# ria8651/octree-tracer

Hardware: AMD Instinct MI355X
Metric: Mrays/sec at 1920x1080, depth-16 SVO; achieved HBM GB/s vs peak (higher is better)
Workload: dtype f32+u32

## Files before the change

include/svo_hip.h:

```cpp
#ifndef SVO_HIP_H
#define SVO_HIP_H

#include <stddef.h>
#include <stdint.h>

#ifdef __cplusplus
extern "C" {
#endif

#define SVO_VOXEL_OFFSET 134217728u

typedef enum svo_status {
    SVO_OK = 0,
    SVO_ERR_ARG = -1,
    SVO_ERR_HIP = -2,
    SVO_ERR_STATE = -3,
    SVO_ERR_NO_DEVICE = -4,
    SVO_ERR_COMM = -5,
    SVO_ERR_CAP = -6
} svo_status;

#define SVO_F_PAUSE_ADAPTIVE 1u
#define SVO_F_SHOW_STEPS 2u
#define SVO_F_SHOW_HITS 4u
// ... 19 lines not shown
typedef struct svo_ctx svo_ctx;

#define SVO_VARIANT_RESTART 0
#define SVO_VARIANT_STACK 1

typedef enum svo_option {
    SVO_OPT_VARIANT = 0,
    SVO_OPT_TIMING = 1,
    SVO_OPT_GRID_BLOCKS = 2,
    SVO_OPT_REFILL_MIN = 3,
    SVO_OPT_STRIP_ITEMS = 4,
    SVO_OPT_DYNAMIC_STRIPS = 5,
    SVO_OPT_SCHEDULE = 8,
    SVO_OPT_TREE_DEPTH = 9,
    SVO_OPT_BLOCK_SHAPE = 10,
    SVO_OPT_DEBUG_BUFFER = 7,
    SVO_OPT_SCAN_CLEARS_COUNTERS = 11,
    SVO_OPT_FUSED_SHADOWS = 12,
    SVO_OPT_PAIR_TABLE = 13,
    SVO_OPT_CULL = 14,
    SVO_OPT_CAMERA_SHORTCUT = 15,
    SVO_OPT_SCHEDULE_MOTION = 16,
    SVO_OPT_STATIC_DEAL = 17,
    SVO_OPT_PRIO_STEPS = 6
} svo_option;

int svo_device_count(void);
int svo_ctx_create(int hip_device, svo_ctx **out);
int svo_ctx_destroy(svo_ctx *ctx);
int svo_ctx_set_stream(svo_ctx *ctx, void *hip_stream, int use_own);
int svo_set_option(svo_ctx *ctx, int option, int64_t value);
const char *svo_last_error(const svo_ctx *ctx);
int svo_sync(svo_ctx *ctx);

int svo_nodes_alloc(svo_ctx *ctx, size_t capacity_words);
int svo_nodes_bind_device(svo_ctx *ctx, uint32_t *device_words, size_t capacity_words);
int svo_nodes_share(svo_ctx *ctx, svo_ctx *owner);
int svo_nodes_invalidate(svo_ctx *ctx);
int svo_nodes_write(svo_ctx *ctx, size_t word_offset, const uint32_t *host_words, size_t n);
int svo_nodes_scatter(svo_ctx *ctx, const uint32_t *indices, const uint32_t *host_words, size_t n);
int svo_nodes_read(svo_ctx *ctx, size_t word_offset, uint32_t *host_words, size_t n);
int svo_nodes_device_ptr(svo_ctx *ctx, uint32_t **out, size_t *capacity_words);

int svo_buffer_alloc(svo_ctx *ctx, size_t bytes, void **device_out);
int svo_buffer_free(svo_ctx *ctx, void *device_ptr);
int svo_buffer_read(svo_ctx *ctx, const void *device_ptr, void *host_out, size_t bytes);
// ... 23 lines not shown
int svo_comm_unique_id(uint8_t id_out[SVO_COMM_ID_BYTES]);
int svo_comm_init_rank(svo_ctx *ctx, const uint8_t id[SVO_COMM_ID_BYTES], int world, int rank);
int svo_comm_init_all(int n, svo_ctx *const *ctxs);
int svo_comm_destroy(svo_ctx *ctx);
int svo_gather_frame(svo_ctx *ctx, const void *send, size_t bytes, void *recv_on_root, int root);
int svo_gather_wait(svo_ctx *ctx);
int svo_gather_frame_all(int n, svo_ctx *const *ctxs, const void *const *send, size_t bytes, void *recv_on_root, int root);

int svo_assemble_tiles_rgba(svo_ctx *ctx, const uint32_t *gathered_rgba, uint32_t world, uint32_t n_pad, uint32_t width,
                            uint32_t height, uint32_t tile_w, uint32_t tile_h, uint32_t *rgba_frame_out);

int svo_trace_rays(svo_ctx *ctx, const float *rays, size_t n_rays, svo_hit *hits_out);

int svo_last_render_ms(svo_ctx *ctx, float *ms);
int svo_timing_collect(svo_ctx *ctx, float *ms_out, size_t cap, size_t *n_out);

int svo_diag_gather(svo_ctx *ctx, uint32_t stride_bytes, uint32_t n_loads);

int svo_diag_strip_classes(svo_ctx *ctx, uint8_t *host_out, size_t n_strips);

int svo_diag_deal(svo_ctx *ctx, uint32_t status_out[16], uint32_t *table_out, size_t table_words, uint32_t *stamps_out,
                  size_t stamps_words);

int svo_scan_dispatch(svo_ctx *ctx, uint32_t node_length);
int svo_scan_read(svo_ctx *ctx, uint32_t *sub, uint32_t *n_sub, uint32_t *unsub, uint32_t *n_unsub,
                  size_t capacity);

struct svo_cpu_octree;
struct svo_world;
typedef struct svo_proc_params {
    float pos[3];
    uint32_t base_depth;
    uint32_t chunk_depth;
    uint64_t max_nodes;
} svo_proc_params;
int svo_proc_generate_chunk(svo_ctx *ctx, const svo_proc_params *params, struct svo_cpu_octree **out);
int svo_world_generate(svo_ctx *ctx, struct svo_world *w, uint32_t world_depth, uint32_t chunk_depth);
int svo_proc_sdf(svo_ctx *ctx, const float *xyz, size_t n, float *out);
int svo_proc_classify(svo_ctx *ctx, const svo_proc_params *params, uint8_t *cells_out);
#define SVO_PROC_TIMES 10
int svo_proc_timing(svo_ctx *ctx, float ms_out[SVO_PROC_TIMES]);

typedef struct svo_build_params {
    uint32_t depth;
    uint32_t default_colour;
    uint64_t max_words;
// ... 111 lines not shown
```

octree-tracer_amd/_lib.py:

```python
import ctypes as C
import os

import torch

_HERE = os.path.dirname(os.path.abspath(__file__))
LIB_PATH = os.environ.get("SVO_HIP_LIB") or os.path.join(_HERE, "libsvo_hip.so")


class Uniforms(C.Structure):
    _fields_ = [
        ("camera", C.c_float * 16),
        ("camera_inverse", C.c_float * 16),
        ("dimensions", C.c_float * 4),
        ("sun_dir", C.c_float * 4),
        ("flags", C.c_uint32),
        ("misc_value", C.c_float),
    ]


class TerrainParams(C.Structure):
    _fields_ = [
        ("seed", C.c_uint32),
        ("max_depth", C.c_uint32),
        ("cam", C.c_float * 3),
# ... 110 lines not shown
    "svo_comm_unique_id": (C.c_int, (vp,)),
    "svo_comm_init_rank": (C.c_int, (vp, vp, C.c_int, C.c_int)),
    "svo_comm_init_all": (C.c_int, (C.c_int, C.POINTER(vp))),
    "svo_comm_destroy": (C.c_int, (vp,)),
    "svo_gather_frame": (C.c_int, (vp, vp, sz, vp, C.c_int)),
    "svo_gather_wait": (C.c_int, (vp,)),
    "svo_gather_frame_all": (C.c_int, (C.c_int, C.POINTER(vp), C.POINTER(vp), sz, vp, C.c_int)),
    "svo_set_uniforms": (C.c_int, (vp, C.POINTER(Uniforms))),
    "svo_render": (C.c_int, (vp, u32, u32, u32, u32, u32, u32, vp, vp)),
    "svo_render_host": (C.c_int, (vp, u32, u32, u32, u32, u32, u32, vp, vp)),
    "svo_render_tiles": (C.c_int, (vp, u32, u32, u32, u32, u32, u32, vp, vp)),
    "svo_render_secondary": (C.c_int, (vp, u32, u32, u32, u32, u32, u32, u32, vp, vp)),
    "svo_render_tiles_secondary": (C.c_int, (vp, u32, u32, u32, u32, u32, u32, u32, vp, vp)),
    "svo_assemble_tiles": (C.c_int, (vp, vp, u32, u32, u32, u32, u32, u32, vp)),
    "svo_assemble_tiles_packed": (C.c_int, (vp, vp, u32, u32, u32, u32, u32, u32, vp)),
    "svo_assemble_tiles_rgba": (C.c_int, (vp, vp, u32, u32, u32, u32, u32, u32, vp)),
    "svo_pack_records": (C.c_int, (vp, vp, sz, vp)),
    "svo_trace_rays": (C.c_int, (vp, vp, sz, vp)),
    "svo_last_render_ms": (C.c_int, (vp, fp)),
    "svo_timing_collect": (C.c_int, (vp, fp, sz, C.POINTER(sz))),
    "svo_diag_gather": (C.c_int, (vp, u32, u32)),
    "svo_diag_strip_classes": (C.c_int, (vp, vp, sz)),
    "svo_diag_deal": (C.c_int, (vp, vp, vp, sz, vp, sz)),
    "svo_scan_dispatch": (C.c_int, (vp, u32)),
    "svo_scan_read": (C.c_int, (vp, vp, C.POINTER(u32), vp, C.POINTER(u32), sz)),
    "svo_proc_generate_chunk": (C.c_int, (vp, C.POINTER(ProcParams), C.POINTER(vp))),
    "svo_world_generate": (C.c_int, (vp, vp, u32, u32)),
    "svo_proc_sdf": (C.c_int, (vp, vp, sz, vp)),
    "svo_proc_classify": (C.c_int, (vp, C.POINTER(ProcParams), vp)),
    "svo_proc_timing": (C.c_int, (vp, fp)),
    "svo_nodes_build": (C.c_int, (vp, vp, vp, sz, C.POINTER(BuildParams), C.POINTER(u64))),
    "svo_nodes_build_dense": (C.c_int, (vp, vp, C.POINTER(BuildParams), C.POINTER(u64))),
    "svo_buffer_write": (C.c_int, (vp, vp, vp, sz)),
    "svo_build_timing": (C.c_int, (vp, fp)),
    "svo_cpu_octree_build": (C.c_int, (vp, vp, vp, sz, C.POINTER(ChunkBuildParams), C.POINTER(vp))),
    "svo_world_build": (C.c_int, (vp, vp, vp, vp, sz, C.POINTER(ChunkBuildParams))),
    "svo_world_build_timing": (C.c_int, (vp, fp)),
    "svo_nodes_edit": (C.c_int, (vp, vp, vp, sz, C.POINTER(EditParams), C.POINTER(u64))),
    "svo_edit_timing": (C.c_int, (vp, fp)),
    "svo_nodes_compact": (C.c_int, (vp, C.POINTER(CompactParams), vp, C.POINTER(u64))),
    "svo_compact_timing": (C.c_int, (vp, fp)),
    "svo_nodes_list_voxels": (C.c_int, (vp, C.POINTER(ListParams), vp, vp, vp, C.POINTER(u64))),
    "svo_list_timing": (C.c_int, (vp, fp)),
    "svo_nodes_sample": (C.c_int, (vp, C.POINTER(SampleParams), vp, sz, vp, vp, vp)),
    "svo_nodes_sample_dense": (C.c_int, (vp, C.POINTER(SampleParams), C.POINTER(u32), C.POINTER(u32), vp)),
    "svo_sample_timing": (C.c_int, (vp, fp)),
# ... 96 lines not shown
```

octree-tracer_amd/csrc/svo_abi.cpp:

```cpp
#include <hip/hip_runtime.h>

#include <array>
#include <cmath>
#include <cstdio>
#include <cstdlib>
#include <cstring>
#include <new>
#include <string>
#include <vector>

#include "svo_ctx.h"

int svo_fail(svo_ctx *ctx, int code, const char *what) {
    if (ctx) ctx->err = what;
    return code;
}

int svo_fail_hip(svo_ctx *ctx, hipError_t e, const char *what) {
    if (ctx) ctx->err = std::string(what) + ": " + hipGetErrorString(e);
    return SVO_ERR_HIP;
}

namespace {

// ... 135 lines not shown
        }();
        HIP_TRY(ctx, hipMemcpyAsync(sc.balance, equal_shares.data(), sizeof(equal_shares), hipMemcpyHostToDevice, ctx->stream));
    }
    a.balance = plan.feed_balance ? sc.balance : nullptr;
    a.order_cap = svo::order_list_cap(n_strips);
    if (f.filtered) {
        const uint8_t *prev = plan.prior_costs ? sc.cost : nullptr;
        if (a.skip)
            HIP_TRY(ctx, svo::launch_schedule_skipping(a, prev, sc.cls_now, sc.order, n_strips, a.order_cap, ctx->stream));
        else
            HIP_TRY(ctx, svo::launch_schedule_culling(a, prev, sc.cls_now, sc.order, n_strips, a.order_cap, ctx->stream));
        a.order = sc.order;
    } else if (plan.stored_lists) {
        a.order = sc.order;
    }
    return SVO_OK;
}

int deal_before(svo_ctx *ctx, svo_ctx::Sched &sc, const svo::FrameFacts &ff, svo::TraceArgs &a, const svo::LaunchInfo &li, int sched_slot,
                svo::DealPlan &plan) {
    svo_ctx::Sched::DealBuffers &db = sc.deal;
    svo::DealFacts f;
    f.enabled = ctx->static_deal;
    f.plain_static = sched_slot == 0 && a.work.mode != 2 && a.hits && !a.skip && !a.count_nodes && !a.shadow_hits && !a.debug && !li.deep_stack;
    f.stored_lists = ff.schedule && !ff.filtered && a.order != nullptr && a.balance != nullptr;
    f.at_rest = sc.built_nodes_version == ctx->store->version && memcmp(&sc.built_uniforms, &ctx->uniforms, sizeof(svo_uniforms)) == 0;
    f.balance_frames = sc.state.balance_frames;
    if (f.enabled && f.plain_static && f.stored_lists && f.at_rest) {
        svo::LaunchInfo ask = li;
        ask.blocks_out = &f.grid_blocks;
        HIP_TRY(ctx, svo::launch_trace(a, ask, ctx->stream));
        f.row_cap = svo::deal_row_cap(a.order_cap, f.grid_blocks);
    }
    if (db.seen_pending && hipEventQuery(db.seen_ev[0]) == hipSuccess) {
        db.seen_pending = false;
        f.seen_fresh = true;
        f.seen_step = db.seen[svo::kDealStep];
        f.seen_verdict = db.seen[svo::kDealVerdict];
    }
    (void)hipGetLastError();
    const bool claimed_before = !db.last_replayed;
    plan = svo::deal_before_trace(db.state, f);
    db.last_replayed = plan.replay;
    if (plan.seed) {
        const size_t rows = (size_t)f.grid_blocks * 4;
        if (int rc = svo_grow(ctx, rows * f.row_cap, &db.table)) return rc;
        if (int rc = svo_grow(ctx, rows, &db.len)) return rc;
        if (int rc = svo_grow(ctx, svo::deal_log_words(f.grid_blocks), &db.log)) return rc;
        if (int rc = svo_grow(ctx, sc.order.size(), &db.lists)) return rc;
        if (db.stamps.size() < 2 * rows) {
            if (int rc = svo_grow(ctx, 2 * rows, &db.stamps)) return rc;
            HIP_TRY(ctx, hipMemsetAsync(db.stamps, 0, db.stamps.size() * sizeof(uint32_t), ctx->stream));
        }
        if (!db.words) {
            HIP_TRY(ctx, db.words.alloc(svo::kDealStateWords));
            HIP_TRY(ctx, db.seen.alloc(svo::kDealStateWords));
            HIP_TRY(ctx, db.seen_ev.create(hipEventDisableTiming));
            HIP_TRY(ctx, hipMemsetAsync(db.words, 0, svo::kDealStateWords * sizeof(uint32_t), ctx->stream));
            memset(db.seen, 0, svo::kDealStateWords * sizeof(uint32_t));
        }
        HIP_TRY(ctx, svo::launch_deal_seed(db.view(a.order_cap, ctx->deal_pairs_div), sc.order, claimed_before ? sc.balance.get() : nullptr, ctx->stream));
    }
    if (plan.replay) {
        a.deal_table = db.table;
        a.deal_row_cap = db.state.row_cap;
        a.deal_stamps = db.stamps;
    }
    return SVO_OK;
}

int schedule_after(svo_ctx *ctx, svo_ctx::Sched &sc, svo::FrameFacts &f, const svo::TraceArgs &a, const svo::LaunchInfo &li,
                   int sched_slot, const svo::DealPlan &deal) {
    f.same_input = (a.work.mode != 2 || sched_slot == 1) && sc.built_nodes_version == ctx->store->version &&
                   memcmp(&sc.built_uniforms, &ctx->uniforms, sizeof(svo_uniforms)) == 0;
    f.moving = sc.have_prev && memcmp(&sc.prev_uniforms, &ctx->uniforms, sizeof(svo_uniforms)) != 0;
    svo::PostPlan plan = svo::plan_after_trace(sc.state, f);
    if (deal.replay) plan.balance_update = 0u;
    HIP_TRY(ctx, svo::launch_post(a, li, plan, sc.buf(), ctx->stream));
    if (sched_slot == 0) {
        svo_ctx::Sched::DealBuffers &db = sc.deal;
        const svo::Deal view = db.view(a.order_cap, ctx->deal_pairs_div);
        if (deal.step) HIP_TRY(ctx, svo::launch_deal_step(view, sc.balance, ctx->stream));
        bool mirror = false;
        if (svo::deal_after_post(db.state, deal, plan.build_lists, mirror)) HIP_TRY(ctx, svo::launch_deal_compare(view, sc.order, ctx->stream));
        if (mirror) {
            HIP_TRY(ctx, hipMemcpyAsync(db.seen, db.words, svo::kDealStateWords * sizeof(uint32_t), hipMemcpyDeviceToHost, ctx->stream));
            HIP_TRY(ctx, hipEventRecord(db.seen_ev[0], ctx->stream));
            db.seen_pending = true;
        }
    }
    sc.prev_uniforms = ctx->uniforms;
    sc.have_prev = true;
    if (plan.rebuild) {
        sc.key = a.work;
        sc.built_uniforms = ctx->uniforms;
        sc.built_nodes_version = ctx->store->version;
    }
    return SVO_OK;
}

int trace_launch(svo_ctx *ctx, const svo::WorkDesc &work, const float *rays, svo_hit *hits, const TraceOpts &opt) {
    int rc = bind(ctx);
    if (rc) return rc;
    const bool want_stack = ctx->variant != SVO_VARIANT_RESTART && ctx->tree_depth <= (uint32_t)svo::stack_max_depth(true);
    if (want_stack) {
// ... 56 lines not shown
        ctx->defer_items = want;
    }
    li.counters = ctx->defer_buf;
    if (ctx->defer_buf) {
        uint32_t *lists = ctx->defer_buf + svo::kCounterWords;
        const size_t stride = ctx->defer_items + 1;
        li.defer = lists + (ctx->frame_parity ? stride : 0);
        li.next_defer_count = lists + (ctx->frame_parity ? 0 : stride);
    }
    svo::DealPlan deal;
    if (stack) {
        rc = deal_before(ctx, sc, f, a, li, opt.sched_slot, deal);
        if (rc) return rc;
    }
    const size_t slot = ctx->ev_slots ? (ctx->ev_count % ctx->ev_slots) : 0;
    const bool timed = ctx->ev_slots && opt.sched_slot == 0;
    if (timed) HIP_TRY(ctx, hipEventRecord(ctx->ev[slot][0], ctx->stream));
    HIP_TRY(ctx, svo::launch_trace(a, li, ctx->stream));
    if (timed) {
        HIP_TRY(ctx, hipEventRecord(ctx->ev[slot][1], ctx->stream));
        ctx->ev_count++;
    }
    if (!stack) return SVO_OK;
    rc = schedule_after(ctx, sc, f, a, li, opt.sched_slot, deal);
    if (rc) return rc;
    ctx->frame_parity ^= 1;
    return SVO_OK;
}

bool fuse_shadow_rays(const svo_ctx *ctx) {
    const bool want = ctx->fused_shadows != 0;
    if (!want || ctx->variant == SVO_VARIANT_RESTART || ctx->tree_depth > (uint32_t)svo::stack_max_depth(true)) return false;
    const float *sd = ctx->uniforms.sun_dir;
    const float sl = sqrtf((sd[0] * sd[0] + sd[1] * sd[1]) + sd[2] * sd[2]);
    for (int k = 0; k < 3; k++) {
        float d = -(sd[k] / sl);
        if (d == 0.0f) d = 0.000001f;
        if (!(fabsf(d) >= 1.0e-11f && fabsf(d) <= 2.0f)) return false;
    }
    return true;
}

int trace_common(svo_ctx *ctx, const svo::WorkDesc &work, const float *rays, svo_hit *hits, uint32_t *rgba) {
    if (!ctx->nodes) return svo_fail(ctx, SVO_ERR_STATE, "svo_nodes_alloc / svo_nodes_bind_device not called");
    if (work.mode != 2 && !ctx->have_uniforms) return svo_fail(ctx, SVO_ERR_STATE, "svo_set_uniforms not called");
    if (!hits && !rgba) return svo_fail(ctx, SVO_ERR_ARG, "both hits_out and rgba_out are NULL");
    if (!rgba) return trace_launch(ctx, work, rays, hits, TraceOpts{});
    if (work.mode == 2) return svo_fail(ctx, SVO_ERR_ARG, "explicit rays have no pixels to shade");
    int rc = bind(ctx);
// ... 310 lines not shown
                return svo_fail(ctx, SVO_ERR_ARG, "schedule motion: class floor (0..12, 0 = off) | radius (0..4) << 8 | min_count (0..80) << 12");
            ctx->motion_floor = (uint32_t)value;
            return SVO_OK;
        case SVO_OPT_CAMERA_SHORTCUT:
            ctx->cam_shortcut = value != 0;
            return SVO_OK;
        case SVO_OPT_CULL:
            if (value < 0 || value > 2) return svo_fail(ctx, SVO_ERR_ARG, "cull: 0 (off), 1 (whenever the camera is outside the cube) or 2 (automatic)");
            ctx->cull_mode = (int)value;
            return SVO_OK;
        case SVO_OPT_PAIR_TABLE:
            return SVO_OK;
        case SVO_OPT_DEBUG_BUFFER:
            ctx->debug_buf = (uint32_t *)(uintptr_t)value;
            return SVO_OK;
        case SVO_OPT_BLOCK_SHAPE:
            if (value < 0 || value > 6) return svo_fail(ctx, SVO_ERR_ARG, "block width log2 must be 0..6");
            ctx->block_w_log2 = (uint32_t)value;
            return SVO_OK;
        case SVO_OPT_PRIO_STEPS:
            if (value < 0 || value > 255) return svo_fail(ctx, SVO_ERR_ARG, "prio_steps must be 0..255");
            return SVO_OK;
        case SVO_OPT_STATIC_DEAL:
            if (value < 0 || value > 1) return svo_fail(ctx, SVO_ERR_ARG, "static deal: 0 (off) or 1 (on)");
            ctx->static_deal = value != 0;
            return SVO_OK;
        default:
            return svo_fail(ctx, SVO_ERR_ARG, "unknown option");
    }
}

const char *svo_last_error(const svo_ctx *ctx) { return ctx ? ctx->err.c_str() : "null ctx"; }

int svo_sync(svo_ctx *ctx) {
    if (!ctx) return SVO_ERR_ARG;
    int rc = bind(ctx);
    if (rc) return rc;
    HIP_TRY(ctx, hipStreamSynchronize(ctx->stream));
    if (ctx->comm_stream) HIP_TRY(ctx, hipStreamSynchronize(ctx->comm_stream));
    uint32_t st = 0;
    HIP_TRY(ctx, hipMemcpy(&st, ctx->status, sizeof(st), hipMemcpyDeviceToHost));
    if (st & 2u) {
        HIP_TRY(ctx, hipMemset(ctx->status, 0, sizeof(uint32_t)));
        return svo_fail(ctx, SVO_ERR_STATE, "fused shadow ray outside the range of the fast arithmetic (set SVO_OPT_FUSED_SHADOWS to 0)");
    }
    if (st & 1u) {
        HIP_TRY(ctx, hipMemset(ctx->status, 0, sizeof(uint32_t)));
        return svo_fail(ctx, SVO_ERR_STATE,
// ... 245 lines not shown
    if ((uint64_t)n_loads * (stride_bytes / 4) > ctx->capacity) return svo_fail(ctx, SVO_ERR_ARG, "pattern exceeds the node buffer");
    int rc = bind(ctx);
    if (rc) return rc;
    HIP_TRY(ctx, svo::launch_diag_gather(ctx->nodes, (uint32_t)ctx->capacity, stride_bytes / 4, n_loads, ctx->status, ctx->stream));
    return SVO_OK;
}

int svo_diag_deal(svo_ctx *ctx, uint32_t status_out[16], uint32_t *table_out, size_t table_words, uint32_t *stamps_out, size_t stamps_words) {
    if (!ctx || !status_out) return SVO_ERR_ARG;
    int rc = bind(ctx);
    if (rc) return rc;
    const svo_ctx::Sched::DealBuffers &db = ctx->sched[0].deal;
    uint32_t words[svo::kDealStateWords] = {};
    HIP_TRY(ctx, hipStreamSynchronize(ctx->stream));
    if (db.words) HIP_TRY(ctx, hipMemcpy(words, db.words, sizeof words, hipMemcpyDeviceToHost));
    const uint32_t rows = db.state.seeded ? db.state.grid_blocks * 4u : 0u;
    const uint32_t out[16] = {(uint32_t)db.state.replayed, (uint32_t)db.state.seeds, words[svo::kDealSeeds], words[svo::kDealMoves],
                              words[svo::kDealStep], words[svo::kDealVerdict], db.state.seeded, db.state.claims, rows, db.state.row_cap,
                              words[svo::kDealBestTime], words[svo::kDealBestSample], words[svo::kDealClaimTime], words[svo::kDealLastTime],
                              words[svo::kDealLastMoves], db.state.learn_left};
    memcpy(status_out, out, sizeof out);
    if (table_out && rows) HIP_TRY(ctx, hipMemcpy(table_out, db.table, std::min(table_words, (size_t)rows * db.state.row_cap) * sizeof(uint32_t), hipMemcpyDeviceToHost));
    if (stamps_out && rows) HIP_TRY(ctx, hipMemcpy(stamps_out, db.stamps, std::min(stamps_words, (size_t)rows * 2) * sizeof(uint32_t), hipMemcpyDeviceToHost));
    return SVO_OK;
}

int svo_diag_strip_classes(svo_ctx *ctx, uint8_t *host_out, size_t n_strips) {
    if (!ctx || (!host_out && n_strips)) return SVO_ERR_ARG;
    const svo_ctx::Sched &sc = ctx->sched[0];
    if (!sc.cls_now || !sc.state.order_filtered) return svo_fail(ctx, SVO_ERR_STATE, "the last pixel frame was traced without a culling pass");
    if (n_strips > sc.cap) return svo_fail(ctx, SVO_ERR_ARG, "more strips than the last frame had");
    int rc = bind(ctx);
    if (rc || n_strips == 0) return rc;
    HIP_TRY(ctx, hipMemcpyAsync(host_out, sc.cls_now, n_strips, hipMemcpyDeviceToHost, ctx->stream));
    HIP_TRY(ctx, hipStreamSynchronize(ctx->stream));
    return SVO_OK;
}

int svo_scan_dispatch(svo_ctx *ctx, uint32_t node_length) {
    if (!ctx) return SVO_ERR_ARG;
    if (!ctx->nodes) return svo_fail(ctx, SVO_ERR_STATE, "svo_nodes_alloc not called");
    int rc = bind(ctx);
    if (rc) return rc;
    if (!ctx->scan_lists) {
        HIP_TRY(ctx, ctx->scan_lists.alloc(2 * kScanCapacity));
        ctx->scan_capacity = kScanCapacity;
// ... 38 lines not shown
```

octree-tracer_amd/csrc/svo_ctx.h:

```cpp
#pragma once
#include <hip/hip_runtime.h>

#include <algorithm>
#include <chrono>
#include <cstdint>
#include <cstring>
#include <memory>
#include <string>
#include <type_traits>
#include <utility>
#include <vector>

#include "svo_deal.h"
#include "svo_device.h"
#include "svo_hip.h"
#include "svo_host.h"


template <typename T, bool kPinned>
struct svo_mem {
    T *p = nullptr;
    size_t n = 0;
    svo_mem() = default;
    svo_mem(svo_mem &&o) noexcept : p(o.p), n(o.n) { o.p = nullptr, o.n = 0; }
// ... 130 lines not shown
    uint32_t refill_min = 32;
    bool scan_clears = false;
    int fused_shadows = 2;
    svo_dev<uint32_t> scatter_buf;
    uint32_t block_w_log2 = 3;
    uint32_t tree_depth = 16;
    struct Sched {
        svo::SchedState state;
        svo_dev<uint8_t> cost, cls_now;
        svo_dev<uint32_t> order, balance;
        size_t cap = 0;
        svo::SchedBuffers buf() const { return {cost, cls_now, order, balance}; }
        svo::WorkDesc key{};
        svo_uniforms built_uniforms{};
        uint64_t built_nodes_version = 0;
        svo_uniforms prev_uniforms{};
        bool have_prev = false;
        struct DealBuffers {
            svo::DealState state;
            svo_dev<uint32_t> table, len, log, lists, stamps, words;
            svo_pinned<uint32_t> seen;
            svo_events<1> seen_ev;
            bool seen_pending = false;
            bool last_replayed = false;
            svo::Deal view(uint32_t order_cap, uint32_t pairs_div) const {
                return {table, len, log, lists, stamps, words, state.row_cap, state.grid_blocks, order_cap, pairs_div};
            }
        };
        DealBuffers deal;
        hipError_t alloc(uint32_t n_strips);
        void release() { *this = Sched{}; }
    };
    Sched sched[2];
    bool static_deal = true;
    uint32_t deal_pairs_div = svo::kDealPairsDiv;
    bool list_balance = true;
    uint32_t motion_floor = 0x1204;
    bool schedule = true;
    uint32_t sched_period = 2;
    int frame_parity = 0;
    svo_dev<svo_hit> shade_hits, shade_shadow;
    svo_dev<float> shade_aux, shade_rays;
    svo_dev<uint8_t> shade_skip;
    uint32_t *debug_buf = nullptr;
    uint32_t strip_items = 64;
    std::vector<svo_events<2>> ev;
    size_t ev_slots = 0, ev_count = 0;
    svo_workspace<svo_proc_state> proc{nullptr, nullptr};
    svo_workspace<svo_build_state> build{nullptr, nullptr};
    svo_workspace<svo_adapt_state> adapt{nullptr, nullptr};
    svo_workspace<svo_edit_state> edit{nullptr, nullptr};
    svo_workspace<svo_compact_state> compact{nullptr, nullptr};
    svo_workspace<svo_list_state> list{nullptr, nullptr};
    svo_workspace<svo_sample_state> sample{nullptr, nullptr};
    svo_workspace<svo_voxelize_state> voxelize{nullptr, nullptr};
    std::string err;
};
// ... 183 lines not shown
```

octree-tracer_amd/csrc/svo_deal.h:

```cpp
#pragma once
#include <cstddef>
#include <cstdint>

#include "svo_sched.h"

#if defined(__HIPCC__) || defined(__CUDACC__)
#define SVO_DEAL_HD __host__ __device__
#else
#define SVO_DEAL_HD
#endif

namespace svo {

constexpr uint32_t kDealLearnFrames = 16;
constexpr uint32_t kDealEnd = 0xFFFFFFFFu;
constexpr uint32_t kDealMaxRow = 256;
constexpr uint32_t kDealMaxListWaves = 1024;
constexpr uint32_t kDealPairsDiv = 16;
constexpr uint32_t kDealBalStart = 9, kDealBalStamps = 19, kDealBalBestTime = 20, kDealBalHead = 32, kDealBalSlots = 4096;

enum : uint32_t {
    kDealStep = 0,
    kDealBestTime = 1,
    kDealBestSample = 2,
    kDealVerdict = 3,
    kDealSeeds = 4,
    kDealMoves = 5,
    kDealLastTime = 6,
    kDealLastMoves = 7,
    kDealClaimTime = 8,
    kDealBestStep = 9,
    kDealTmpTime = 16,
    kDealTmpSample = 17,
    kDealTmpMoves = 18,
    kDealStateWords = 32
};

struct Deal {
    uint32_t *table;
    uint32_t *len;
    uint32_t *log;
    uint32_t *lists;
    uint32_t *stamps;
    uint32_t *state;
    uint32_t row_cap, grid_blocks, order_cap, pairs_div;
};

SVO_DEAL_HD inline uint32_t deal_list_waves(uint32_t grid_blocks, uint32_t l) { return ((grid_blocks + 7u - l) / 8u) * 4u; }
SVO_DEAL_HD inline uint32_t deal_wave(uint32_t l, uint32_t rank) { return ((rank >> 2) * 8u + l) * 4u + (rank & 3u); }
SVO_DEAL_HD inline uint32_t deal_log_slot(uint32_t grid_blocks, uint32_t s, uint32_t l, uint32_t p) {
    uint32_t before = 0u;
    for (uint32_t k = 0; k < l; k++) before += deal_list_waves(grid_blocks, k) / 2u;
    return s * (grid_blocks * 2u) + before + p;
}
// ... 174 lines not shown
    if (is_best) {
        d.state[kDealBestTime] = t_frame;
        d.state[kDealBestSample] = d.state[kDealTmpSample];
        d.state[kDealBestStep] = n;
    }
    d.state[kDealStep] = n + 1u;
    if (n + 1u == kDealLearnFrames) {
        const uint32_t learnt = bal[kDealBalBestTime], recent = d.state[kDealClaimTime], ours = d.state[kDealBestSample];
        const uint32_t claims = learnt != 0u && (recent == 0u || learnt < recent) ? learnt : recent;
        d.state[kDealVerdict] = (ours != 0u && (claims == 0u || ours < claims)) ? 1u : 2u;
    }
}


struct DealFacts {
    bool enabled = false;
    bool plain_static = false;
    bool stored_lists = false;
    bool at_rest = false;
    uint32_t balance_frames = 0;
    uint32_t grid_blocks = 0, row_cap = 0;
    uint32_t seen_step = 0, seen_verdict = 0;
    bool seen_fresh = false;
};

struct DealState {
    bool seeded = false;
    bool claims = false;
    uint32_t learn_left = 0;
    uint32_t grid_blocks = 0, row_cap = 0;
    bool want_mirror = false;
    uint64_t replayed = 0, seeds = 0;
};

struct DealPlan {
    bool seed = false;
    bool replay = false;
    bool step = false;
    bool mirror = false;
};

inline DealPlan deal_before_trace(DealState &s, const DealFacts &f) {
    DealPlan p;
    const bool settled = f.at_rest && f.balance_frames >= kBalanceLearnFrames;
    if (!(f.enabled && f.plain_static && f.stored_lists && settled && f.row_cap != 0u)) {
        const uint64_t replayed = s.replayed, seeds = s.seeds;
        s = DealState{};
        s.replayed = replayed;
        s.seeds = seeds;
        return p;
    }
    if (f.seen_fresh && s.want_mirror) {
        s.want_mirror = false;
        if (f.seen_verdict == 2u) s.claims = true;
        if (f.seen_step >= kDealLearnFrames) s.learn_left = 0;
    }
    if (!s.seeded || s.grid_blocks != f.grid_blocks || s.row_cap != f.row_cap) {
        s.seeded = true;
        s.claims = false;
        s.learn_left = kDealLearnFrames;
        s.grid_blocks = f.grid_blocks;
        s.row_cap = f.row_cap;
        s.want_mirror = false;
        s.seeds++;
        p.seed = true;
    }
    if (s.claims) return p;
    p.replay = true;
    s.replayed++;
    if (s.learn_left != 0u) {
        p.step = true;
        s.learn_left--;
        if (s.learn_left == 0u) p.mirror = s.want_mirror = true;
    }
    return p;
}

inline bool deal_after_post(DealState &s, const DealPlan &p, bool lists_rebuilt, bool &mirror) {
    mirror = p.mirror;
    if (!(s.seeded && lists_rebuilt)) return false;
    if (!s.claims) {
        s.learn_left = kDealLearnFrames;
        mirror = s.want_mirror = true;
    }
    return !s.claims;
}

}
```

octree-tracer_amd/csrc/svo_deal.hip:

```cpp
#include <hip/hip_runtime.h>

#include "svo_deal.h"
#include "svo_device.h"

namespace svo {

static_assert(kDealBalStart == kBalanceStart && kDealBalStamps == kBalanceStamps && kDealBalBestTime == kBalanceBestTime &&
                  kDealBalHead == kBalanceHead && kDealBalSlots == kBalanceSlots,
              "svo_deal.h reads the balance words by svo_device.h's numbers");

constexpr uint32_t kDealThreads = 1024;

struct BlockSync {
    __device__ void operator()() const { __syncthreads(); }
};

__global__ __launch_bounds__(kDealThreads) void deal_seed_kernel(Deal d, const uint32_t *order, const uint32_t *bal) {
    __shared__ uint32_t red[kDealThreads];
    deal_seed(d, order, bal, red, threadIdx.x, kDealThreads, BlockSync{});
}

__global__ __launch_bounds__(kDealThreads) void deal_compare_kernel(Deal d, const uint32_t *order) {
    __shared__ uint32_t flag;
    deal_reseed_if_changed(d, order, &flag, threadIdx.x, kDealThreads, BlockSync{});
}

__global__ __launch_bounds__(kDealThreads) void deal_step_kernel(Deal d, const uint32_t *bal) {
    __shared__ uint32_t scratch[2 * kDealMaxListWaves + kDealThreads];
    deal_step(d, bal, scratch, blockIdx.x, threadIdx.x, kDealThreads, BlockSync{});
}

__global__ __launch_bounds__(64) void deal_commit_kernel(Deal d, const uint32_t *bal) {
    if (threadIdx.x == 0u) deal_commit(d, bal);
}

hipError_t launch_deal_seed(const Deal &d, const uint32_t *order, const uint32_t *bal, hipStream_t stream) {
    (void)hipGetLastError();
    hipLaunchKernelGGL(deal_seed_kernel, dim3(1), dim3(kDealThreads), 0, stream, d, order, bal);
    return hipGetLastError();
}

hipError_t launch_deal_compare(const Deal &d, const uint32_t *order, hipStream_t stream) {
    (void)hipGetLastError();
    hipLaunchKernelGGL(deal_compare_kernel, dim3(1), dim3(kDealThreads), 0, stream, d, order);
    return hipGetLastError();
}

hipError_t launch_deal_step(const Deal &d, const uint32_t *bal, hipStream_t stream) {
    (void)hipGetLastError();
    hipLaunchKernelGGL(deal_step_kernel, dim3(8), dim3(kDealThreads), 0, stream, d, bal);
    hipLaunchKernelGGL(deal_commit_kernel, dim3(1), dim3(64), 0, stream, d, bal);
    return hipGetLastError();
}

}
```

octree-tracer_amd/csrc/svo_device.h:

```cpp
#pragma once
#include <hip/hip_runtime.h>
#include <stdint.h>

#include "svo_hip.h"
#include "svo_sched.h"

namespace svo {

constexpr uint32_t kVoxelOffset = 134217728u;
constexpr uint32_t kMaxDescent = 31;
constexpr int kTopLevels = 3;
constexpr int kTopEntries = 1 << (3 * kTopLevels);
constexpr int kTopAuxEntries = 8 + 64;
constexpr int kPathBits = 23;
#ifndef SVO_COUNTER_STRIDE
#define SVO_COUNTER_STRIDE 16416
#endif
constexpr int kCounterStride = SVO_COUNTER_STRIDE;
constexpr int kCounterWords = 64 * kCounterStride;


struct WorkDesc {
    uint32_t mode;
    uint32_t x0, y0;
// ... 54 lines not shown
#ifndef SVO_COST_SHIFT
#define SVO_COST_SHIFT 2
#endif
constexpr uint32_t kCostShift = SVO_COST_SHIFT, kCostClasses = 128u >> SVO_COST_SHIFT;
constexpr uint32_t kOrderHistWords = 64 * kCostClasses;
constexpr uint32_t kBalanceStart = 9;
constexpr uint32_t kBalanceUpdates = 18;
constexpr uint32_t kBalanceStamps = 19;
constexpr uint32_t kBalanceBestTime = 20;
constexpr uint32_t kBalanceBestShares = 21;
constexpr uint32_t kBalanceHead = 32, kBalanceSlots = 4096, kBalanceWords = kBalanceHead + kBalanceSlots;
inline uint32_t order_list_cap(uint32_t n_strips) { return (n_strips + 3u) / 4u + kCostClasses; }
struct SchedBuffers {
    uint8_t *cost;
    uint8_t *cls_now;
    uint32_t *order;
    uint32_t *balance;
};
hipError_t launch_post(const TraceArgs &args, const LaunchInfo &li, const PostPlan &plan, const SchedBuffers &buf, hipStream_t stream);
hipError_t launch_build_lists(const TraceArgs &args, uint32_t motion_floor, const SchedBuffers &buf, hipStream_t stream);

struct Deal;
hipError_t launch_deal_seed(const Deal &d, const uint32_t *order, const uint32_t *bal, hipStream_t stream);
hipError_t launch_deal_step(const Deal &d, const uint32_t *bal, hipStream_t stream);
hipError_t launch_deal_compare(const Deal &d, const uint32_t *order, hipStream_t stream);

hipError_t launch_schedule_skipping(const TraceArgs &args, const uint8_t *prev, uint8_t *cls, uint32_t *sched, uint32_t n_strips,
                                    uint32_t cap, hipStream_t stream);
hipError_t launch_schedule_culling(const TraceArgs &args, const uint8_t *prev, uint8_t *cls, uint32_t *sched, uint32_t n_strips,
                                   uint32_t cap, hipStream_t stream);
hipError_t launch_secondary_gen(const TraceArgs &args, const float *aux_t, float *rays, uint8_t *skip, svo_hit *out, uint32_t k_first,
                                uint32_t n_secondary, uint32_t n_records, hipStream_t stream);
hipError_t launch_shade(const TraceArgs &args, const svo_hit *shadow_hits, uint32_t *rgba, hipStream_t stream);
hipError_t launch_diag_gather(const uint32_t *buf, uint32_t n_words, uint32_t stride_words, uint32_t n_loads, uint32_t *sink,
                              hipStream_t stream);
hipError_t launch_scan(uint32_t *nodes, uint32_t n_words, uint32_t node_length, uint32_t *sub, uint32_t *unsub,
                       uint32_t capacity, bool clear_counters, hipStream_t stream);
hipError_t launch_assemble_tiles(const void *gathered, bool packed, svo_hit *frame, uint32_t world, uint32_t n_pad, uint32_t width,
                                 uint32_t height, uint32_t tile_w, uint32_t tile_h, hipStream_t stream);
hipError_t launch_assemble_tiles_rgba(const uint32_t *gathered, uint32_t *frame, uint32_t world, uint32_t n_pad, uint32_t width,
                                      uint32_t height, uint32_t tile_w, uint32_t tile_h, hipStream_t stream);
hipError_t launch_pack_records(const svo_hit *records, uint32_t *wire, uint32_t n, hipStream_t stream);
hipError_t launch_scatter(uint32_t *nodes, uint32_t n_words, const uint32_t *indices, const uint32_t *words, uint32_t n,
                          hipStream_t stream);

}
```

octree-tracer_amd/gpu.py:

```python
import ctypes as C

import torch

from ._lib import SvoError, lib

OPT_VARIANT, OPT_TIMING, OPT_GRID_BLOCKS, OPT_REFILL_MIN, OPT_STRIP_ITEMS, OPT_DYNAMIC_STRIPS, OPT_PRIO_STEPS, OPT_DEBUG_BUFFER, OPT_SCHEDULE, OPT_TREE_DEPTH, OPT_BLOCK_SHAPE, OPT_SCAN_CLEARS_COUNTERS, OPT_FUSED_SHADOWS, OPT_PAIR_TABLE, OPT_CULL, OPT_CAMERA_SHORTCUT, OPT_SCHEDULE_MOTION, OPT_STATIC_DEAL = range(18)
VARIANT_RESTART, VARIANT_STACK = 0, 1


class Gpu:
    def __init__(self, device=0, stream=None):
        h = C.c_void_p()
        rc = lib().svo_ctx_create(device, C.byref(h))
        if rc != 0:
            raise SvoError(f"svo_ctx_create(device={device}) failed with status {rc} (no usable HIP device?)")
        self._h = h
        self.device = device
        self.torch_device = torch.device("cuda", device)
        self.tree_depth = 16
        self.set_stream(stream if stream is not None else torch.cuda.current_stream(device).cuda_stream)

    @classmethod
    def new(cls, device=0):
        return cls(device)

    def check(self, rc):
        if rc != 0:
            raise SvoError(f"status {rc}: {lib().svo_last_error(self._h).decode()}")

# ... 52 lines not shown
        self.check(lib().svo_diag_strip_classes(self._h, out.ctypes.data_as(C.c_void_p), n_strips))
        return out

    DEAL_STATUS = ("replayed", "seeds", "device_seeds", "moves", "step", "verdict", "seeded", "claims", "rows", "row_cap",
                   "best_ticks", "best_sample_ticks", "claim_ticks", "last_ticks", "last_moves", "learn_left")

    def deal_status(self, table=False, stamps=False):
        import numpy as np
        st = np.zeros(16, dtype=np.uint32)
        self.check(lib().svo_diag_deal(self._h, st.ctypes.data_as(C.c_void_p), None, 0, None, 0))
        out = dict(zip(self.DEAL_STATUS, (int(v) for v in st)))
        rows, cap = out["rows"], out["row_cap"]
        tab = np.zeros((rows, cap), dtype=np.uint32) if table else None
        stp = np.zeros((rows, 2), dtype=np.uint32) if stamps else None
        if rows and (table or stamps):
            self.check(lib().svo_diag_deal(self._h, st.ctypes.data_as(C.c_void_p), tab.ctypes.data_as(C.c_void_p) if table else None,
                                           tab.size if table else 0, stp.ctypes.data_as(C.c_void_p) if stamps else None, stp.size if stamps else 0))
        if table:
            out["table"] = tab
        if stamps:
            out["stamps"] = stp
        return out

    def timing_collect(self, cap=65536):
        import numpy as np
        buf = np.empty(cap, dtype=np.float32)
        n = C.c_size_t()
        self.check(lib().svo_timing_collect(self._h, buf.ctypes.data_as(C.POINTER(C.c_float)), cap, C.byref(n)))
        return buf[:n.value].copy()

    @staticmethod
    def comm_unique_id():
        buf = (C.c_uint8 * 128)()
        rc = lib().svo_comm_unique_id(buf)
        if rc != 0:
            raise SvoError(f"svo_comm_unique_id failed with status {rc} (librccl missing?)")
        return bytes(buf)

    def comm_init_rank(self, unique_id, world, rank):
        buf = (C.c_uint8 * 128).from_buffer_copy(unique_id)
        self.check(lib().svo_comm_init_rank(self._h, buf, world, rank))

    @staticmethod
    def comm_init_all(gpus):
        arr = (C.c_void_p * len(gpus))(*[g._h for g in gpus])
        rc = lib().svo_comm_init_all(len(gpus), arr)
# ... 22 lines not shown
```

Before: 10870.

## Skip post-trace pass when static deal replay is settled and idle

Adds an idle-post mode, on by default, that skips the per-frame post pass and deal bookkeeping once static deal replay has finished learning. This applies only when the verdict stays on replay, no rays were deferred, and nothing needs rebuilding or rebalancing. The deal commit kernel now records a deferred count so the host can tell when skipping is safe. The aim is to remove a kernel launch and its memory traffic from each steady-state frame. The risk is stale schedule state if the scene changes without tripping one of the guards.

```diff
diff --git a/include/svo_hip.h b/include/svo_hip.h
--- a/include/svo_hip.h
+++ b/include/svo_hip.h
@@ -65,6 +65,7 @@
     SVO_OPT_CAMERA_SHORTCUT = 15,
     SVO_OPT_SCHEDULE_MOTION = 16,
     SVO_OPT_STATIC_DEAL = 17,
+    SVO_OPT_IDLE_POST = 18,
     SVO_OPT_PRIO_STEPS = 6
 } svo_option;
 
@@ -134,6 +135,8 @@
 int svo_diag_deal(svo_ctx *ctx, uint32_t status_out[16], uint32_t *table_out, size_t table_words, uint32_t *stamps_out,
                   size_t stamps_words);
 
+int svo_diag_post(svo_ctx *ctx, uint32_t out[4]);
+
 int svo_scan_dispatch(svo_ctx *ctx, uint32_t node_length);
 int svo_scan_read(svo_ctx *ctx, uint32_t *sub, uint32_t *n_sub, uint32_t *unsub, uint32_t *n_unsub,
                   size_t capacity);
diff --git a/octree-tracer_amd/_lib.py b/octree-tracer_amd/_lib.py
--- a/octree-tracer_amd/_lib.py
+++ b/octree-tracer_amd/_lib.py
@@ -156,6 +156,7 @@
     "svo_diag_gather": (C.c_int, (vp, u32, u32)),
     "svo_diag_strip_classes": (C.c_int, (vp, vp, sz)),
     "svo_diag_deal": (C.c_int, (vp, vp, vp, sz, vp, sz)),
+    "svo_diag_post": (C.c_int, (vp, vp)),
     "svo_scan_dispatch": (C.c_int, (vp, u32)),
     "svo_scan_read": (C.c_int, (vp, vp, C.POINTER(u32), vp, C.POINTER(u32), sz)),
     "svo_proc_generate_chunk": (C.c_int, (vp, C.POINTER(ProcParams), C.POINTER(vp))),
diff --git a/octree-tracer_amd/csrc/svo_abi.cpp b/octree-tracer_amd/csrc/svo_abi.cpp
--- a/octree-tracer_amd/csrc/svo_abi.cpp
+++ b/octree-tracer_amd/csrc/svo_abi.cpp
@@ -181,6 +181,7 @@
     svo_ctx::Sched::DealBuffers &db = sc.deal;
     svo::DealFacts f;
     f.enabled = ctx->static_deal;
+    f.force_replay = ctx->deal_force_replay;
     f.plain_static = sched_slot == 0 && a.work.mode != 2 && a.hits && !a.skip && !a.count_nodes && !a.shadow_hits && !a.debug && !li.deep_stack;
     f.stored_lists = ff.schedule && !ff.filtered && a.order != nullptr && a.balance != nullptr;
     f.at_rest = sc.built_nodes_version == ctx->store->version && memcmp(&sc.built_uniforms, &ctx->uniforms, sizeof(svo_uniforms)) == 0;
@@ -196,6 +197,7 @@
         f.seen_fresh = true;
         f.seen_step = db.seen[svo::kDealStep];
         f.seen_verdict = db.seen[svo::kDealVerdict];
+        f.seen_deferred = db.seen_deferred = db.seen[svo::kDealDeferred];
     }
     (void)hipGetLastError();
     const bool claimed_before = !db.last_replayed;
@@ -229,17 +231,23 @@
 }
 
 int schedule_after(svo_ctx *ctx, svo_ctx::Sched &sc, svo::FrameFacts &f, const svo::TraceArgs &a, const svo::LaunchInfo &li,
-                   int sched_slot, const svo::DealPlan &deal) {
+                   int sched_slot, const svo::DealPlan &deal, bool &post_skipped) {
     f.same_input = (a.work.mode != 2 || sched_slot == 1) && sc.built_nodes_version == ctx->store->version &&
                    memcmp(&sc.built_uniforms, &ctx->uniforms, sizeof(svo_uniforms)) == 0;
     f.moving = sc.have_prev && memcmp(&sc.prev_uniforms, &ctx->uniforms, sizeof(svo_uniforms)) != 0;
     svo::PostPlan plan = svo::plan_after_trace(sc.state, f);
     if (deal.replay) plan.balance_update = 0u;
-    HIP_TRY(ctx, svo::launch_post(a, li, plan, sc.buf(), ctx->stream));
-    if (sched_slot == 0) {
+    post_skipped = sched_slot == 0 && ctx->idle_post && svo::deal_skips_post(sc.deal.state, deal, plan);
+    if (post_skipped) {
+        ctx->posts_skipped++;
+    } else {
+        HIP_TRY(ctx, svo::launch_post(a, li, plan, sc.buf(), ctx->stream));
+        ctx->posts_launched++;
+    }
+    if (sched_slot == 0 && !post_skipped) {
         svo_ctx::Sched::DealBuffers &db = sc.deal;
         const svo::Deal view = db.view(a.order_cap, ctx->deal_pairs_div);
-        if (deal.step) HIP_TRY(ctx, svo::launch_deal_step(view, sc.balance, ctx->stream));
+        if (deal.step) HIP_TRY(ctx, svo::launch_deal_step(view, sc.balance, li.defer, ctx->stream));
         bool mirror = false;
         if (svo::deal_after_post(db.state, deal, plan.build_lists, mirror)) HIP_TRY(ctx, svo::launch_deal_compare(view, sc.order, ctx->stream));
         if (mirror) {
@@ -342,9 +350,10 @@
         ctx->ev_count++;
     }
     if (!stack) return SVO_OK;
-    rc = schedule_after(ctx, sc, f, a, li, opt.sched_slot, deal);
-    if (rc) return rc;
-    ctx->frame_parity ^= 1;
+    bool post_skipped = false;
+    rc = schedule_after(ctx, sc, f, a, li, opt.sched_slot, deal, post_skipped);
+    if (rc) return rc;
+    if (!post_skipped) ctx->frame_parity ^= 1;
     return SVO_OK;
 }
 
@@ -701,8 +710,14 @@
             if (value < 0 || value > 255) return svo_fail(ctx, SVO_ERR_ARG, "prio_steps must be 0..255");
             return SVO_OK;
         case SVO_OPT_STATIC_DEAL:
-            if (value < 0 || value > 1) return svo_fail(ctx, SVO_ERR_ARG, "static deal: 0 (off) or 1 (on)");
+            if (value < 0 || value > 2) return svo_fail(ctx, SVO_ERR_ARG, "static deal: 0 (off), 1 (on) or 2 (on, never back to claims)");
             ctx->static_deal = value != 0;
+            if ((value == 2) != ctx->deal_force_replay) ctx->sched[0].deal.state.seeded = false;
+            ctx->deal_force_replay = value == 2;
+            return SVO_OK;
+        case SVO_OPT_IDLE_POST:
+            if (value < 0 || value > 1) return svo_fail(ctx, SVO_ERR_ARG, "idle post: 0 (every STACK frame launches its post pass) or 1");
+            ctx->idle_post = value != 0;
             return SVO_OK;
         default:
             return svo_fail(ctx, SVO_ERR_ARG, "unknown option");
@@ -994,6 +1009,16 @@
     memcpy(status_out, out, sizeof out);
     if (table_out && rows) HIP_TRY(ctx, hipMemcpy(table_out, db.table, std::min(table_words, (size_t)rows * db.state.row_cap) * sizeof(uint32_t), hipMemcpyDeviceToHost));
     if (stamps_out && rows) HIP_TRY(ctx, hipMemcpy(stamps_out, db.stamps, std::min(stamps_words, (size_t)rows * 2) * sizeof(uint32_t), hipMemcpyDeviceToHost));
+    return SVO_OK;
+}
+
+int svo_diag_post(svo_ctx *ctx, uint32_t out[4]) {
+    if (!ctx || !out) return SVO_ERR_ARG;
+    const svo_ctx::Sched::DealBuffers &db = ctx->sched[0].deal;
+    out[0] = ctx->posts_launched;
+    out[1] = ctx->posts_skipped;
+    out[2] = db.state.post_idle;
+    out[3] = db.seen_deferred;
     return SVO_OK;
 }
 
diff --git a/octree-tracer_amd/csrc/svo_ctx.h b/octree-tracer_amd/csrc/svo_ctx.h
--- a/octree-tracer_amd/csrc/svo_ctx.h
+++ b/octree-tracer_amd/csrc/svo_ctx.h
@@ -176,6 +176,7 @@
             svo_pinned<uint32_t> seen;
             svo_events<1> seen_ev;
             bool seen_pending = false;
+            uint32_t seen_deferred = 0;
             bool last_replayed = false;
             svo::Deal view(uint32_t order_cap, uint32_t pairs_div) const {
                 return {table, len, log, lists, stamps, words, state.row_cap, state.grid_blocks, order_cap, pairs_div};
@@ -187,6 +188,9 @@
     };
     Sched sched[2];
     bool static_deal = true;
+    bool deal_force_replay = false;
+    bool idle_post = true;
+    uint32_t posts_launched = 0, posts_skipped = 0;
     uint32_t deal_pairs_div = svo::kDealPairsDiv;
     bool list_balance = true;
     uint32_t motion_floor = 0x1204;
diff --git a/octree-tracer_amd/csrc/svo_deal.h b/octree-tracer_amd/csrc/svo_deal.h
--- a/octree-tracer_amd/csrc/svo_deal.h
+++ b/octree-tracer_amd/csrc/svo_deal.h
@@ -30,6 +30,7 @@
     kDealLastMoves = 7,
     kDealClaimTime = 8,
     kDealBestStep = 9,
+    kDealDeferred = 10,
     kDealTmpTime = 16,
     kDealTmpSample = 17,
     kDealTmpMoves = 18,
@@ -250,6 +251,8 @@
     uint32_t grid_blocks = 0, row_cap = 0;
     uint32_t seen_step = 0, seen_verdict = 0;
     bool seen_fresh = false;
+    uint32_t seen_deferred = 0;
+    bool force_replay = false;
 };
 
 struct DealState {
@@ -258,6 +261,7 @@
     uint32_t learn_left = 0;
     uint32_t grid_blocks = 0, row_cap = 0;
     bool want_mirror = false;
+    bool post_idle = false;
     uint64_t replayed = 0, seeds = 0;
 };
 
@@ -280,8 +284,10 @@
     }
     if (f.seen_fresh && s.want_mirror) {
         s.want_mirror = false;
-        if (f.seen_verdict == 2u) s.claims = true;
+        if (f.seen_verdict == 2u && !f.force_replay) s.claims = true;
         if (f.seen_step >= kDealLearnFrames) s.learn_left = 0;
+        const bool stays_on_replay = f.seen_verdict == 1u || (f.seen_verdict == 2u && f.force_replay);
+        s.post_idle = f.seen_step >= kDealLearnFrames && stays_on_replay && f.seen_deferred == 0u;
     }
     if (!s.seeded || s.grid_blocks != f.grid_blocks || s.row_cap != f.row_cap) {
         s.seeded = true;
@@ -290,6 +296,7 @@
         s.grid_blocks = f.grid_blocks;
         s.row_cap = f.row_cap;
         s.want_mirror = false;
+        s.post_idle = false;
         s.seeds++;
         p.seed = true;
     }
@@ -307,6 +314,7 @@
 inline bool deal_after_post(DealState &s, const DealPlan &p, bool lists_rebuilt, bool &mirror) {
     mirror = p.mirror;
     if (!(s.seeded && lists_rebuilt)) return false;
+    s.post_idle = false;
     if (!s.claims) {
         s.learn_left = kDealLearnFrames;
         mirror = s.want_mirror = true;
@@ -314,4 +322,8 @@
     return !s.claims;
 }
 
-}
+inline bool deal_skips_post(const DealState &s, const DealPlan &p, const PostPlan &post) {
+    return p.replay && s.post_idle && !p.step && !p.mirror && !p.seed && !post.rebuild && !post.build_lists && post.balance_update == 0u;
+}
+
+}
diff --git a/octree-tracer_amd/csrc/svo_deal.hip b/octree-tracer_amd/csrc/svo_deal.hip
--- a/octree-tracer_amd/csrc/svo_deal.hip
+++ b/octree-tracer_amd/csrc/svo_deal.hip
@@ -30,8 +30,11 @@
     deal_step(d, bal, scratch, blockIdx.x, threadIdx.x, kDealThreads, BlockSync{});
 }
 
-__global__ __launch_bounds__(64) void deal_commit_kernel(Deal d, const uint32_t *bal) {
-    if (threadIdx.x == 0u) deal_commit(d, bal);
+__global__ __launch_bounds__(64) void deal_commit_kernel(Deal d, const uint32_t *bal, const uint32_t *deferred) {
+    if (threadIdx.x == 0u) {
+        deal_commit(d, bal);
+        d.state[kDealDeferred] = *deferred;
+    }
 }
 
 hipError_t launch_deal_seed(const Deal &d, const uint32_t *order, const uint32_t *bal, hipStream_t stream) {
@@ -46,10 +49,10 @@
     return hipGetLastError();
 }
 
-hipError_t launch_deal_step(const Deal &d, const uint32_t *bal, hipStream_t stream) {
+hipError_t launch_deal_step(const Deal &d, const uint32_t *bal, const uint32_t *deferred, hipStream_t stream) {
     (void)hipGetLastError();
     hipLaunchKernelGGL(deal_step_kernel, dim3(8), dim3(kDealThreads), 0, stream, d, bal);
-    hipLaunchKernelGGL(deal_commit_kernel, dim3(1), dim3(64), 0, stream, d, bal);
+    hipLaunchKernelGGL(deal_commit_kernel, dim3(1), dim3(64), 0, stream, d, bal, deferred);
     return hipGetLastError();
 }
 
diff --git a/octree-tracer_amd/csrc/svo_device.h b/octree-tracer_amd/csrc/svo_device.h
--- a/octree-tracer_amd/csrc/svo_device.h
+++ b/octree-tracer_amd/csrc/svo_device.h
@@ -100,7 +100,7 @@
 
 struct Deal;
 hipError_t launch_deal_seed(const Deal &d, const uint32_t *order, const uint32_t *bal, hipStream_t stream);
-hipError_t launch_deal_step(const Deal &d, const uint32_t *bal, hipStream_t stream);
+hipError_t launch_deal_step(const Deal &d, const uint32_t *bal, const uint32_t *deferred, hipStream_t stream);
 hipError_t launch_deal_compare(const Deal &d, const uint32_t *order, hipStream_t stream);
 
 hipError_t launch_schedule_skipping(const TraceArgs &args, const uint8_t *prev, uint8_t *cls, uint32_t *sched, uint32_t n_strips,
diff --git a/octree-tracer_amd/gpu.py b/octree-tracer_amd/gpu.py
--- a/octree-tracer_amd/gpu.py
+++ b/octree-tracer_amd/gpu.py
@@ -4,7 +4,7 @@
 
 from ._lib import SvoError, lib
 
-OPT_VARIANT, OPT_TIMING, OPT_GRID_BLOCKS, OPT_REFILL_MIN, OPT_STRIP_ITEMS, OPT_DYNAMIC_STRIPS, OPT_PRIO_STEPS, OPT_DEBUG_BUFFER, OPT_SCHEDULE, OPT_TREE_DEPTH, OPT_BLOCK_SHAPE, OPT_SCAN_CLEARS_COUNTERS, OPT_FUSED_SHADOWS, OPT_PAIR_TABLE, OPT_CULL, OPT_CAMERA_SHORTCUT, OPT_SCHEDULE_MOTION, OPT_STATIC_DEAL = range(18)
+OPT_VARIANT, OPT_TIMING, OPT_GRID_BLOCKS, OPT_REFILL_MIN, OPT_STRIP_ITEMS, OPT_DYNAMIC_STRIPS, OPT_PRIO_STEPS, OPT_DEBUG_BUFFER, OPT_SCHEDULE, OPT_TREE_DEPTH, OPT_BLOCK_SHAPE, OPT_SCAN_CLEARS_COUNTERS, OPT_FUSED_SHADOWS, OPT_PAIR_TABLE, OPT_CULL, OPT_CAMERA_SHORTCUT, OPT_SCHEDULE_MOTION, OPT_STATIC_DEAL, OPT_IDLE_POST = range(19)
 VARIANT_RESTART, VARIANT_STACK = 0, 1
 
 
@@ -103,6 +103,14 @@
             out["stamps"] = stp
         return out
 
+    POST_STATUS = ("launched", "skipped", "post_idle", "deferred")
+
+    def post_status(self):
+        import numpy as np
+        st = np.zeros(4, dtype=np.uint32)
+        self.check(lib().svo_diag_post(self._h, st.ctypes.data_as(C.c_void_p)))
+        return dict(zip(self.POST_STATUS, (int(v) for v in st)))
+
     def timing_collect(self, cap=65536):
         import numpy as np
         buf = np.empty(cap, dtype=np.float32)
```

New measurement: 10920, median of 2. About the same (+0.4%).
